# XinMing0411/zero-shot-AAC

Hardware: AMD Instinct MI355X
Metric: audio clips/sec end-to-end (encode+mapper+GPT-2 decode), Clotho-eval bs=64 (higher is better)
Workload: dtype bf16

## Files before the change

zero-shot-aac_amd/csrc/gemm.hip:

```cpp
#include <algorithm>
#include "gemm_fast.h"

namespace zs {

int g_gemm_fast = 1;
int g_gemm_dbg = 0;
int g_fast_xcd = 1;

__device__ __forceinline__ void store_out(void* out, int out_dtype, long idx, float v) {
  if (out_dtype == ZS_BF16) reinterpret_cast<bf16_t*>(out)[idx] = f2bf(v);
  else reinterpret_cast<float*>(out)[idx] = v;
}

template <typename T, int BM, int BN>
__global__ __launch_bounds__(256) void gemm_kernel(GemmArgs g) {
  constexpr int LDW = BK + GemmTraits<T>::PAD;
  __shared__ __attribute__((aligned(16))) T smem[2 * (BM + BN) * LDW];
  constexpr int TM = BM / 64, TN = BN / 64;
  const int n0 = blockIdx.x * BN, m0 = blockIdx.y * BM, z = blockIdx.z;
  const int kbeg = z * g.k_per_split, kend = min(g.K, kbeg + g.k_per_split);
  f32x16_t acc[TM][TN];
  DenseA<T, BM> la{(const T*)g.A, g.lda, g.M, m0};
  gemm_mainloop<T, BM, BN>(la, (const T*)g.W, g.ldw, g.N, n0, kbeg, kend, smem, acc);
  const int lane = threadIdx.x & 63, wid = threadIdx.x >> 6;
  const int wr0 = (wid >> 1) * (BM / 2), wc0 = (wid & 1) * (BN / 2);
#pragma unroll
  for (int i = 0; i < TM; ++i)
#pragma unroll
    for (int j = 0; j < TN; ++j) {
      const int n = n0 + wc0 + j * 32 + (lane & 31);
      if (n >= g.N) continue;
      const float bias = (g.split_k == 1 && g.bias) ? g.bias[n] : 0.f;
#pragma unroll
      for (int e = 0; e < 16; ++e) {
        const int m = m0 + wr0 + i * 32 + (e & 3) + 8 * (e >> 2) + 4 * (lane >> 5);
        if (m >= g.M) continue;
        float v = acc[i][j][e];
        if (g.split_k > 1) {
          g.ws[((long)z * g.M + m) * g.N + n] = v;
        } else {
          v = act_apply(v + bias, g.act);
          if (g.residual) v += g.residual[(long)m * g.ldr + n];
          store_out(g.out, g.out_dtype, (long)m * g.ldo + n, v);
        }
      }
    }
}

__global__ void splitk_reduce_kernel(GemmArgs g) {
  long idx = (long)blockIdx.x * blockDim.x + threadIdx.x;
  long total = (long)g.M * g.N;
  if (idx >= total) return;
  int m = idx / g.N, n = idx % g.N;
  float v = 0.f;
  for (int z = 0; z < g.split_k; ++z) v += g.ws[(long)z * total + idx];
  if (g.bias) v += g.bias[n];
  v = act_apply(v, g.act);
  if (g.residual) v += g.residual[(long)m * g.ldr + n];
  store_out(g.out, g.out_dtype, (long)m * g.ldo + n, v);
}

template <int ACT, int WN>
__device__ __forceinline__ void epi_slab(const GemmArgs& g, const float* slab, int mr0, int nc0,
                                         int z, bool vec_out, bool vec_res, const float (&bb)[8],
                                         const float4 (&res)[WN / 16][2]) {
  constexpr int Q = WN / 8, IT = 32 * Q / 64;
  static_assert(IT * 64 == 32 * Q, "slab iterations");
  const int lane = threadIdx.x & 63;
#pragma unroll
  for (int it = 0; it < IT; ++it) {
    const int idx = lane + 64 * it;
    const int r = idx / Q, c = (idx % Q) * 8;
    const int m = mr0 + r, n = nc0 + c;
    if (m >= g.M || n >= g.N) continue;
    const float4 a0 = *reinterpret_cast<const float4*>(slab + r * WN + c);
    const float4 a1 = *reinterpret_cast<const float4*>(slab + r * WN + c + 4);
    float v[8] = {a0.x, a0.y, a0.z, a0.w, a1.x, a1.y, a1.z, a1.w};
    const int nv = min(8, g.N - n);
    const bool full = nv == 8;
    if (g.split_k > 1) {
      float* dst = g.ws + ((long)z * g.M + m) * g.N + n;
      if (full && g.N % 4 == 0) {
        reinterpret_cast<float4*>(dst)[0] = make_float4(v[0], v[1], v[2], v[3]);
        reinterpret_cast<float4*>(dst)[1] = make_float4(v[4], v[5], v[6], v[7]);
      } else {
        for (int q = 0; q < nv; ++q) dst[q] = v[q];
      }
      continue;
    }
    if constexpr (64 % Q == 0) {
#pragma unroll
      for (int q = 0; q < 8; ++q) v[q] = act_apply_fast(v[q] + bb[q], ACT);
    } else {
#pragma unroll
      for (int q = 0; q < 8; ++q)
        v[q] = act_apply_fast(v[q] + ((g.bias && q < nv) ? g.bias[n + q] : 0.f), ACT);
    }
    if (g.residual) {
      if (full && vec_res) {
        const float4 r0 = res[it][0], r1 = res[it][1];
        v[0] += r0.x; v[1] += r0.y; v[2] += r0.z; v[3] += r0.w;
        v[4] += r1.x; v[5] += r1.y; v[6] += r1.z; v[7] += r1.w;
      } else {
        const float* rp = g.residual + (long)m * g.ldr + n;
        for (int q = 0; q < nv; ++q) v[q] += rp[q];
      }
    }
    const long o = (long)m * g.ldo + n;
    if (full && vec_out) {
      if (g.out_dtype == ZS_BF16) {
        uint4 u;
        u.x = pk2bf(v[0], v[1]);
        u.y = pk2bf(v[2], v[3]);
        u.z = pk2bf(v[4], v[5]);
        u.w = pk2bf(v[6], v[7]);
        if (g.dbg != 6 || u.x == 0x7fc17fc1u)
          *reinterpret_cast<uint4*>(reinterpret_cast<bf16_t*>(g.out) + o) = u;
      } else {
        float4* d = reinterpret_cast<float4*>(reinterpret_cast<float*>(g.out) + o);
        d[0] = make_float4(v[0], v[1], v[2], v[3]);
        d[1] = make_float4(v[4], v[5], v[6], v[7]);
      }
    } else {
      for (int q = 0; q < nv; ++q) store_out(g.out, g.out_dtype, o + q, v[q]);
    }
  }
}

template <int WN>
__device__ __forceinline__ void epi_res_load(const GemmArgs& g, int mr0, int nc0, bool vec_res,
                                             float4 (&res)[WN / 16][2]) {
  constexpr int Q = WN / 8, IT = 32 * Q / 64;
  const int lane = threadIdx.x & 63;
#pragma unroll
  for (int it = 0; it < IT; ++it) {
    const int idx = lane + 64 * it;
    const int m = mr0 + idx / Q, n = nc0 + (idx % Q) * 8;
    if (g.residual && vec_res && g.split_k == 1 && m < g.M && n + 8 <= g.N) {
      const float4* rp = reinterpret_cast<const float4*>(g.residual + (long)m * g.ldr + n);
      res[it][0] = rp[0];
      res[it][1] = rp[1];
    } else {
      res[it][0] = res[it][1] = make_float4(0.f, 0.f, 0.f, 0.f);
    }
  }
}

template <int BM, int BN, int NS, int WGM, int WGN, int BK_, bool F32 = false>
__global__ __launch_bounds__(64 * WGM * WGN,
                             (WGM * WGN == 4 && NS * FastTile<BM, BN, WGM, WGN, BK_>::STAGE <= 80 * 1024)
                                 ? 2 : 1) void gemm_fast_kernel(GemmArgs g) {
  constexpr int KF = F32 ? 2 : 1;
  using FT = FastTile<BM, BN, WGM, WGN, BK_>;
  __shared__ __attribute__((aligned(16))) char lds[NS * FT::STAGE];
  constexpr int TM = FT::TM, TN = FT::TN, WN = FT::WN;
  if (g.dbg == 5) return;
  static_assert(FT::NW * 32 * WN * 4 <= NS * FT::STAGE, "epilogue slab must fit the stage ring");
  const int ntn = cdiv(g.N, BN), ntm = cdiv(g.M, BM);
  const int ntiles = ntn * ntm * g.split_k;
// ... 87 lines not shown
      for (int q = 0; q < WN / 16; ++q) { res[q][0] = res0[q][0]; res[q][1] = res0[q][1]; }
    } else {
      epi_res_load<WN>(g, mr0, nc0, vec_res, res);
    }
#pragma unroll
    for (int j = 0; j < TN; ++j)
#pragma unroll
      for (int e = 0; e < 16; ++e)
        slab[((e & 3) + 8 * (e >> 2) + 4 * (lane >> 5)) * WN + j * 32 + (lane & 31)] = acc[i][j][e];
    switch (g.act) {
      case ACT_GELU_ERF: epi_slab<ACT_GELU_ERF, WN>(g, slab, mr0, nc0, cz, vec_out, vec_res, bb, res); break;
      case ACT_GELU_TANH: epi_slab<ACT_GELU_TANH, WN>(g, slab, mr0, nc0, cz, vec_out, vec_res, bb, res); break;
      case ACT_RELU: epi_slab<ACT_RELU, WN>(g, slab, mr0, nc0, cz, vec_out, vec_res, bb, res); break;
      case ACT_TANH: epi_slab<ACT_TANH, WN>(g, slab, mr0, nc0, cz, vec_out, vec_res, bb, res); break;
      default: epi_slab<ACT_NONE, WN>(g, slab, mr0, nc0, cz, vec_out, vec_res, bb, res); break;
    }
  }
  asm volatile("s_waitcnt lgkmcnt(0)" ::: "memory");
  __builtin_amdgcn_s_barrier();
  }
}

template <int BM, int BN, int NS, int BK_, int WGM = 2, int WGN = 2>
__global__ __launch_bounds__(64 * WGM * WGN, WGM * WGN == 4 ? 2 : 1) void gemm_lean_kernel(GemmArgs g) {
  using FT = FastTile<BM, BN, WGM, WGN, BK_>;
  constexpr int TM = FT::TM, TN = FT::TN, WN = FT::WN, NW = WGM * WGN;
  static_assert(NW * 32 * WN * 4 <= NS * FT::STAGE, "epilogue slab fits the ring");
  __shared__ __attribute__((aligned(16))) char lds[NS * FT::STAGE];
  const int ntn = cdiv(g.N, BN), ntm = cdiv(g.M, BM), ntiles = ntn * ntm;
  int m0, n0;
  {
    const int b = blockIdx.x, x = b & 7, q8 = ntiles >> 3, r8 = ntiles & 7;
    const int u = (x < r8 ? x * (q8 + 1) : r8 * (q8 + 1) + (x - r8) * q8) + (b >> 3);
    const int conc = max(1, min(q8, 64));
    int gm = (int)(sqrtf((float)conc * BN / BM) + 0.5f);
    gm = max(1, min(gm, ntm));
    const int per = gm * ntn, grp = u / per, fm = grp * gm;
    const int gs = min(ntm - fm, gm), r = u - grp * per;
    m0 = (fm + r % gs) * BM;
    n0 = (r / gs) * BN;
  }
  const int lane = threadIdx.x & 63, wid = threadIdx.x >> 6;
  f32x16_t acc[TM][TN];
  lean_mainloop<BM, BN, NS, WGM, WGN, BK_, false, true>((const bf16_t*)g.A, g.lda, g.M, m0,
                                                        (const bf16_t*)g.W, g.ldw, g.N, n0, g.K,
                                                        lds, acc);
  const int wr0 = (wid / WGN) * FT::WM, wc0 = (wid % WGN) * WN;
  const bool vec_out = g.ldo % 8 == 0 && ((uintptr_t)g.out & 15) == 0;
  const bool vec_res = g.residual == nullptr || (g.ldr % 4 == 0 && ((uintptr_t)g.residual & 15) == 0);
  float bb[8];
  {
    const int n = n0 + wc0 + (lane % (WN / 8)) * 8, nv = min(8, g.N - n);
    if (g.bias && nv == 8 && ((uintptr_t)(g.bias + n) & 15) == 0) {
      const float4 b0 = reinterpret_cast<const float4*>(g.bias + n)[0];
      const float4 b1 = reinterpret_cast<const float4*>(g.bias + n)[1];
      bb[0] = b0.x; bb[1] = b0.y; bb[2] = b0.z; bb[3] = b0.w;
      bb[4] = b1.x; bb[5] = b1.y; bb[6] = b1.z; bb[7] = b1.w;
    } else {
#pragma unroll
      for (int q = 0; q < 8; ++q) bb[q] = (g.bias && q < nv) ? g.bias[n + q] : 0.f;
    }
  }
  float* slab = reinterpret_cast<float*>(lds) + wid * 32 * WN;
#pragma unroll
  for (int i = 0; i < TM; ++i) {
    const int mr0 = m0 + wr0 + i * 32, nc0 = n0 + wc0;
    float4 res[WN / 16][2];
    epi_res_load<WN>(g, mr0, nc0, vec_res, res);
#pragma unroll
    for (int j = 0; j < TN; ++j)
#pragma unroll
      for (int e = 0; e < 16; ++e)
        slab[((e & 3) + 8 * (e >> 2) + 4 * (lane >> 5)) * WN + j * 32 + (lane & 31)] = acc[i][j][e];
    switch (g.act) {
      case ACT_GELU_ERF: epi_slab<ACT_GELU_ERF, WN>(g, slab, mr0, nc0, 0, vec_out, vec_res, bb, res); break;
      case ACT_GELU_TANH: epi_slab<ACT_GELU_TANH, WN>(g, slab, mr0, nc0, 0, vec_out, vec_res, bb, res); break;
      case ACT_RELU: epi_slab<ACT_RELU, WN>(g, slab, mr0, nc0, 0, vec_out, vec_res, bb, res); break;
      case ACT_TANH: epi_slab<ACT_TANH, WN>(g, slab, mr0, nc0, 0, vec_out, vec_res, bb, res); break;
      default: epi_slab<ACT_NONE, WN>(g, slab, mr0, nc0, 0, vec_out, vec_res, bb, res); break;
    }
  }
}

namespace big {
constexpr int BM = 256, BN = 256, BKB = 64, RB = 128, BUF = (BM + BN) * RB;
__device__ __forceinline__ int swz(int row) { return (row >> 1) & 7; }
__device__ __forceinline__ int set_instr(int set, int j) {
  if (set < 2) return ((j >> 3) * 128 + set * 64) / 8 + (j & 7);
  return (BM + (j >> 2) * 64 + (set - 2) * 32) / 8 + (j & 3);
}
}

typedef __attribute__((ext_vector_type(4))) float f32x4_t;
template <int ACT>
__device__ __forceinline__ void big_epilogue(const GemmArgs& g, float* slab, int mrw, int nc0,
                                             bool vec_out, bool vec_res, const float (&bb)[8],
                                             const f32x4_t (&acc)[8][4]) {
  const int lane = threadIdx.x & 63, fr = lane & 15, fq = lane >> 4;
#pragma unroll
  for (int sl = 0; sl < 4; ++sl) {
    const int mr0 = mrw + 32 * sl;
    float4 res[4][2];
    epi_res_load<64>(g, mr0, nc0, vec_res, res);
#pragma unroll
    for (int ii = 0; ii < 2; ++ii)
#pragma unroll
      for (int j = 0; j < 4; ++j)
#pragma unroll
        for (int e = 0; e < 4; ++e)
          slab[(16 * ii + 4 * fq + e) * 64 + 16 * j + fr] = acc[2 * sl + ii][j][e];
    epi_slab<ACT, 64>(g, slab, mr0, nc0, 0, vec_out, vec_res, bb, res);
  }
}

__global__ __launch_bounds__(512) void gemm_big_kernel(GemmArgs g) {
  using namespace big;
  __shared__ __attribute__((aligned(16))) char lds[2 * BUF];
  const int ntn = cdiv(g.N, BN), ntm = cdiv(g.M, BM), ntiles = ntn * ntm;
  int m0, n0;
  {
    const int b = blockIdx.x, x = b & 7, q8 = ntiles >> 3, r8 = ntiles & 7;
    const int u = (x < r8 ? x * (q8 + 1) : r8 * (q8 + 1) + (x - r8) * q8) + (b >> 3);
    const int conc = max(1, min(q8, 32));
    int gm = (int)(sqrtf((float)conc) + 0.5f);
    gm = max(1, min(gm, ntm));
    const int per = gm * ntn, grp = u / per, fm = grp * gm;
    const int gs = min(ntm - fm, gm), r = u - grp * per;
    m0 = (fm + r % gs) * BM;
    n0 = (r / gs) * BN;
  }
  const int lane = threadIdx.x & 63, wid = threadIdx.x >> 6, wr = wid >> 2, wc = wid & 3;
  const bf16_t* A = (const bf16_t*)g.A;
  const bf16_t* W = (const bf16_t*)g.W;
  int src[4][2];
#pragma unroll
  for (int set = 0; set < 4; ++set)
#pragma unroll
    for (int jj = 0; jj < 2; ++jj) {
      const int idx = set_instr(set, wid + 8 * jj);
      const int row = 8 * idx + (lane >> 3);
      const int c = 8 * ((lane & 7) ^ swz(row));
      src[set][jj] = set < 2 ? min(m0 + row, g.M - 1) * g.lda + c
                             : min(n0 + row - BM, g.N - 1) * g.ldw + c;
    }
  auto issue = [&](int set, char* bufp, int k0) {
#pragma unroll
    for (int jj = 0; jj < 2; ++jj)
      __builtin_amdgcn_global_load_lds((gptr_t)((set < 2 ? A : W) + src[set][jj] + k0),
                                       (lds_ptr_t)(bufp + set_instr(set, wid + 8 * jj) * 1024),
                                       16, 0, 0);
  };
  auto tile_issue = [&](char* bufp, int k0) {
    issue(0, bufp, k0); issue(2, bufp, k0); issue(3, bufp, k0); issue(1, bufp, k0);
  };
  f32x4_t acc[8][4];
#pragma unroll
  for (int i = 0; i < 8; ++i)
#pragma unroll
    for (int j = 0; j < 4; ++j) acc[i][j] = f32x4_t{0.f, 0.f, 0.f, 0.f};
  const int nk = g.K / BKB;
  tile_issue(lds, 0);
  if (nk > 1) tile_issue(lds + BUF, BKB);
  const int fr = lane & 15, fq = lane >> 4;
  const int arow = wr * 128 + fr, brow = BM + wc * 64 + fr;
  int aoff[2], boff[2];
#pragma unroll
  for (int s2 = 0; s2 < 2; ++s2) {
    aoff[s2] = arow * RB + 16 * ((4 * s2 + fq) ^ swz(arow));
    boff[s2] = brow * RB + 16 * ((4 * s2 + fq) ^ swz(brow));
  }
  bf16x8_t a[4][2], b0[2][2], b1[2][2];
#pragma unroll 1
  for (int t = 0; t < nk; ++t) {
    char* bufp = lds + (t & 1) * BUF;
    const bool pf = t + 2 < nk;
    const int kn = (t + 2) * BKB;
// ... 38 lines not shown
          acc[i][2 + j] = __builtin_amdgcn_mfma_f32_16x16x32_bf16(a[i][s2], b1[j][s2], acc[i][2 + j], 0, 0, 0);
    __builtin_amdgcn_s_setprio(0);
    if (pf) wait_vm<12>(); else if (t + 2 == nk) wait_vm<8>(); else wait_vm<0>();
    __builtin_amdgcn_s_barrier();
    asm volatile("" ::: "memory");
#pragma unroll
    for (int i = 0; i < 4; ++i)
#pragma unroll
      for (int s2 = 0; s2 < 2; ++s2)
        a[i][s2] = *reinterpret_cast<const bf16x8_t*>(bufp + aoff[s2] + 2048 * (4 + i));
    if (pf) issue(3, bufp, kn);
    __builtin_amdgcn_s_setprio(1);
#pragma unroll
    for (int s2 = 0; s2 < 2; ++s2)
#pragma unroll
      for (int i = 0; i < 4; ++i)
#pragma unroll
        for (int j = 0; j < 2; ++j)
          acc[4 + i][2 + j] = __builtin_amdgcn_mfma_f32_16x16x32_bf16(a[i][s2], b1[j][s2], acc[4 + i][2 + j], 0, 0, 0);
    __builtin_amdgcn_s_setprio(0);
    __builtin_amdgcn_s_barrier();
    asm volatile("" ::: "memory");
    if (pf) issue(1, bufp, kn);
    __builtin_amdgcn_s_setprio(1);
#pragma unroll
    for (int s2 = 0; s2 < 2; ++s2)
#pragma unroll
      for (int i = 0; i < 4; ++i)
#pragma unroll
        for (int j = 0; j < 2; ++j)
          acc[4 + i][j] = __builtin_amdgcn_mfma_f32_16x16x32_bf16(a[i][s2], b0[j][s2], acc[4 + i][j], 0, 0, 0);
    __builtin_amdgcn_s_setprio(0);
  }
  wait_vm<0>();
  __syncthreads();
  const bool vec_out = g.ldo % 8 == 0 && ((uintptr_t)g.out & 15) == 0;
  const bool vec_res = g.residual == nullptr || (g.ldr % 4 == 0 && ((uintptr_t)g.residual & 15) == 0);
  const int nc0 = n0 + wc * 64;
  float bb[8];
  {
    const int n = nc0 + (lane % 8) * 8, nv = min(8, g.N - n);
    if (g.bias && nv == 8 && ((uintptr_t)(g.bias + n) & 15) == 0) {
      const float4 c0 = reinterpret_cast<const float4*>(g.bias + n)[0];
      const float4 c1 = reinterpret_cast<const float4*>(g.bias + n)[1];
      bb[0] = c0.x; bb[1] = c0.y; bb[2] = c0.z; bb[3] = c0.w;
      bb[4] = c1.x; bb[5] = c1.y; bb[6] = c1.z; bb[7] = c1.w;
    } else {
#pragma unroll
      for (int q = 0; q < 8; ++q) bb[q] = (g.bias && q < nv) ? g.bias[n + q] : 0.f;
    }
  }
  float* slab = reinterpret_cast<float*>(lds) + wid * 32 * 64;
  const int mrw = m0 + wr * 128;
  switch (g.act) {
    case ACT_GELU_ERF: big_epilogue<ACT_GELU_ERF>(g, slab, mrw, nc0, vec_out, vec_res, bb, acc); break;
    case ACT_GELU_TANH: big_epilogue<ACT_GELU_TANH>(g, slab, mrw, nc0, vec_out, vec_res, bb, acc); break;
    case ACT_RELU: big_epilogue<ACT_RELU>(g, slab, mrw, nc0, vec_out, vec_res, bb, acc); break;
    case ACT_TANH: big_epilogue<ACT_TANH>(g, slab, mrw, nc0, vec_out, vec_res, bb, acc); break;
    default: big_epilogue<ACT_NONE>(g, slab, mrw, nc0, vec_out, vec_res, bb, acc); break;
  }
}

int g_gemm_big = 1;
int g_big_min = 256;

static int launch_big(GemmArgs& g, hipStream_t st) {
  hipLaunchKernelGGL(gemm_big_kernel, dim3(cdiv(g.N, 256) * cdiv(g.M, 256)), dim3(512), 0, st, g);
  ZS_LAUNCH_CHECK();
  return 0;
}

int g_gemm_lean = 1;
int g_lean96 = 0;
int g_lean8w = 0;

template <int BM, int BN, int NS, int BK_, int WGM = 2, int WGN = 2>
static int launch_lean(GemmArgs& g, hipStream_t st) {
  hipLaunchKernelGGL((gemm_lean_kernel<BM, BN, NS, BK_, WGM, WGN>),
                     dim3(cdiv(g.N, BN) * cdiv(g.M, BM)), dim3(64 * WGM * WGN), 0, st, g);
  ZS_LAUNCH_CHECK();
  return 0;
}

int g_fast_persist = 1;

template <int BM, int BN, int NS, int WGM = 2, int WGN = 2, int BK_ = 64, bool F32 = false>
static int launch_fast(GemmArgs& g, hipStream_t st) {
  using FT = FastTile<BM, BN, WGM, WGN, BK_>;
  const long nt = (long)cdiv(g.N, BN) * cdiv(g.M, BM) * g.split_k;
  const int per_cu = max(1, min(160 * 1024 / (NS * FT::STAGE), 8 / FT::NW * 2));
  dim3 grid(g_fast_persist ? (int)std::min<long>(nt, 256L * per_cu) : (int)nt);
  hipLaunchKernelGGL((gemm_fast_kernel<BM, BN, NS, WGM, WGN, BK_, F32>), grid,
                     dim3(64 * WGM * WGN), 0, st, g);
  ZS_LAUNCH_CHECK();
  return 0;
}

static long nblocks(const GemmArgs& g, int bm, int bn) {
  return (long)cdiv(g.M, bm) * cdiv(g.N, bn) * g.split_k;
}

int g_fast_ns = 2;
int g_fast_tile = 0;
int g_lean_min128 = 256;
#ifndef ZS_LEAN128_NS
#define ZS_LEAN128_NS 3
#endif
int g_lean128_ns = ZS_LEAN128_NS;

static int dispatch_fast(GemmArgs& g, hipStream_t st) {
  switch (g_fast_tile) {
    case 1: return launch_fast<256, 256, 4, 2, 4, 32>(g, st);
    case 2: return launch_fast<256, 128, 4, 4, 2, 32>(g, st);
    case 3: return launch_fast<128, 256, 4, 2, 4, 32>(g, st);
    case 4: return launch_fast<128, 128, 2>(g, st);
    case 5: return launch_fast<128, 128, 4, 2, 2, 32>(g, st);
    case 6: return launch_fast<256, 256, 2, 2, 4, 64>(g, st);
    case 7: return launch_fast<128, 128, 6, 2, 2, 32>(g, st);
    case 8: return launch_fast<128, 64, 3>(g, st);
    case 9: return launch_fast<64, 128, 3>(g, st);
    case 10: return launch_fast<128, 128, 3>(g, st);
    case 11: return launch_fast<128, 128, 2, 2, 2, 32>(g, st);
    case 12: return launch_fast<128, 128, 3, 2, 2, 32>(g, st);
    case 13: return launch_fast<64, 64, 2>(g, st);
    case 14: return launch_fast<128, 128, 4>(g, st);
    case 15: return launch_fast<256, 128, 2, 4, 2, 64>(g, st);
    case 16: return launch_fast<128, 256, 2, 2, 4, 64>(g, st);
    case 17: return launch_fast<64, 64, 2, 2, 2, 128>(g, st);
    default: break;
  }
  if ((g_fast_tile == 18 || (g_gemm_big && g.K >= 2048 && nblocks(g, 256, 256) >= g_big_min)) &&
      g.split_k == 1 && g.K % 64 == 0 && g.lda % 8 == 0 && g.ldw % 8 == 0)
    return launch_big(g, st);
  if (g_gemm_lean && g.split_k == 1 && g.K % 64 == 0) {
    const int lt = g_fast_tile >= 100 ? g_fast_tile - 100 : 0;
    const long n128 = nblocks(g, 128, 128);
    if (!lt && g_lean8w && g.N >= 3072 && n128 >= 1024 && n128 <= 4096)
      return launch_lean<256, 128, 3, 64, 2, 4>(g, st);
    if (!lt && g_lean96 && g.N % 96 == 0 && g.N <= 1536 && nblocks(g, 128, 96) >= 384)
      return launch_lean<128, 96, 2, 64, 4, 1>(g, st);
    if (lt == 1 || (!lt && n128 >= g_lean_min128)) return launch_lean<128, 128, 2, 64>(g, st);
    if (!lt && n128 >= 128)
      return g_lean128_ns == 4 ? launch_lean<128, 128, 4, 64, 2, 4>(g, st)
                               : launch_lean<128, 128, 3, 64, 2, 4>(g, st);
    if (lt == 2 || (!lt && nblocks(g, 128, 64) >= 256))
      return g.M >= g.N ? launch_lean<128, 64, 3, 64>(g, st) : launch_lean<64, 128, 3, 64>(g, st);
    if ((lt == 3 || (!lt && g.M >= 512 && nblocks(g, 64, 64) < 256)) && g.K % 128 == 0)
      return launch_lean<64, 64, 2, 128>(g, st);
    if (lt == 5) return launch_lean<256, 128, 2, 64, 4, 2>(g, st);
    if (lt == 6) return launch_lean<128, 256, 2, 64, 2, 4>(g, st);
    if (lt == 7) return launch_lean<256, 256, 2, 64, 2, 4>(g, st);
    if (lt == 8) return launch_lean<256, 128, 3, 64, 4, 2>(g, st);
    if (lt == 9) return launch_lean<128, 256, 3, 64, 2, 4>(g, st);
    if (lt == 10) return launch_lean<256, 128, 3, 64, 2, 4>(g, st);
    if (lt == 11) return launch_lean<128, 128, 3, 64, 2, 4>(g, st);
    if (lt == 12) return launch_lean<128, 128, 4, 64, 2, 4>(g, st);
    if (lt == 13) return launch_lean<128, 96, 2, 64, 4, 1>(g, st);
    return launch_lean<64, 64, 4, 64>(g, st);
  }
  if (nblocks(g, 128, 128) >= 256) {
    if (g_fast_ns == 3) return launch_fast<128, 128, 3>(g, st);
    if (g_fast_ns == 4) return launch_fast<128, 128, 4>(g, st);
    return launch_fast<128, 128, 2>(g, st);
  }
  if (nblocks(g, 128, 64) >= 256) return g.M >= g.N ? launch_fast<128, 64, 3>(g, st)
                                                     : launch_fast<64, 128, 3>(g, st);
  if (g.k_per_split % 128 == 0) return launch_fast<64, 64, 2, 2, 2, 128>(g, st);
  return launch_fast<64, 64, 4>(g, st);
}

template <typename T, int BM, int BN>
static int launch_gemm(GemmArgs& g, hipStream_t st) {
  dim3 grid(cdiv(g.N, BN), cdiv(g.M, BM), g.split_k);
  hipLaunchKernelGGL((gemm_kernel<T, BM, BN>), grid, dim3(256), 0, st, g);
  ZS_LAUNCH_CHECK();
  return 0;
}

int g_f32_fast = 1;
int g_f32_tile = 8;
static int dispatch_fast_f32(GemmArgs& g, hipStream_t st) {
  if (g_f32_tile >= 7) {
    if (nblocks(g, 128, 128) >= 256) {
      if (g_f32_tile == 10) return launch_fast<128, 128, 2, 2, 2, 128, true>(g, st);
      if (g_f32_tile == 11 && nblocks(g, 256, 128) >= 256)
        return launch_fast<256, 128, 2, 4, 2, 64, true>(g, st);
      return g_f32_tile == 7 ? launch_fast<128, 128, 2, 2, 4, 64, true>(g, st)
                             : launch_fast<128, 128, 2, 2, 2, 64, true>(g, st);
    }
    if (nblocks(g, 128, 64) >= 256)
      return g.M >= g.N ? launch_fast<128, 64, 2, 2, 2, 64, true>(g, st)
                        : launch_fast<64, 128, 2, 2, 2, 64, true>(g, st);
    return launch_fast<64, 64, 2, 2, 2, 64, true>(g, st);
  }
  if (g_f32_tile && nblocks(g, 128, 128) >= 256) {
    switch (g_f32_tile) {
      case 1: return launch_fast<128, 128, 3, 2, 2, 64, true>(g, st);
      case 2: return launch_fast<128, 128, 2, 2, 2, 64, true>(g, st);
      case 3: return launch_fast<256, 128, 4, 4, 2, 32, true>(g, st);
      case 4: return launch_fast<128, 256, 4, 2, 4, 32, true>(g, st);
      case 5: return launch_fast<128, 128, 6, 2, 2, 32, true>(g, st);
      case 6: return launch_fast<128, 128, 4, 2, 4, 32, true>(g, st);
      default: break;
    }
  }
  if (nblocks(g, 128, 128) >= 256) return launch_fast<128, 128, 4, 2, 2, 32, true>(g, st);
  if (nblocks(g, 128, 64) >= 256)
    return g.M >= g.N ? launch_fast<128, 64, 4, 2, 2, 32, true>(g, st)
                      : launch_fast<64, 128, 4, 2, 2, 32, true>(g, st);
  return launch_fast<64, 64, 4, 2, 2, 32, true>(g, st);
}

template <typename T>
static int dispatch_gemm(GemmArgs& g, hipStream_t st) {
  if (sizeof(T) == 2 && g_gemm_fast) return dispatch_fast(g, st);
  if (sizeof(T) == 4 && g_f32_fast && g.K % 4 == 0 && g.lda % 4 == 0 && g.ldw % 4 == 0 &&
      g.k_per_split % 4 == 0 && ((uintptr_t)g.A & 15) == 0 && ((uintptr_t)g.W & 15) == 0)
    return dispatch_fast_f32(g, st);
  const bool small_m = g.M <= 64;
  const bool wide_n = g.N >= 2048 && !small_m;
  if (small_m) return wide_n ? launch_gemm<T, 64, 128>(g, st) : launch_gemm<T, 64, 64>(g, st);
  if (wide_n) return launch_gemm<T, 128, 128>(g, st);
  return launch_gemm<T, 128, 64>(g, st);
}

}

using namespace zs;

extern "C" __attribute__((visibility("hidden"))) int zs_gemm_skinny_internal(
    int M, int N, int K, int dtype, const void* A, int lda, const void* W, int ldw,
    const float* bias, const float* residual, int ldr, void* out, int ldo, int out_dtype, int act,
    float* workspace, void* stream);

extern "C" __attribute__((visibility("hidden"))) int zs_gemm_rows_internal(
    int M, int N, int K, const void* A, int lda, const void* W, int ldw, const float* bias,
    const float* residual, int ldr, void* out, int ldo, int out_dtype, int act, void* stream);

extern "C" int zs_gemm(int M, int N, int K, int dtype, const void* A, int lda, const void* W,
                       int ldw, const float* bias, const float* residual, int ldr, void* out,
// ... 44 lines not shown
```

zero-shot-aac_amd/csrc/gemm_skinny.hip:

```cpp
#include <cstring>
#include "common.h"

namespace zs {

typedef __attribute__((ext_vector_type(8))) __bf16 bf16x8s_t;
typedef __attribute__((ext_vector_type(16))) float f32x16s_t;

constexpr int SK_BN = 32;
constexpr int SK_TILE = 64 * SK_BN;
constexpr int SK_MAX_TILES = 4096;
constexpr int SK_MAX_M = 256;

struct SkinnyArgs {
  int M, N, K, lda, ldw, ldr, ldo, splits, ks;
  int rblocks, ntiles;
  const void* A;
  const void* W;
  const float* bias;
  const float* residual;
  void* out;
  int out_dtype, act;
  int* counters;
  float* slabs;
};
// ... 118 lines not shown
  }
  const int ntiles = g.ntiles;
  float* slabs = g.slabs + (long)rb * g.splits * ntiles * SK_TILE;
  int* counter = g.counters + rb * ntiles + tile;
  const long slab_off = ((long)z * ntiles + tile) * SK_TILE + e0;
  __amdgpu_buffer_rsrc_t rsrc = __builtin_amdgcn_make_buffer_rsrc(
      slabs, (short)0, g.splits * ntiles * SK_TILE * 4, 0x00020000);
  if (MODE == 1) {
#pragma unroll
    for (int q = 0; q < PER / 4; ++q) {
      u32x4_t v = {__float_as_uint(part[4 * q]), __float_as_uint(part[4 * q + 1]),
                   __float_as_uint(part[4 * q + 2]), __float_as_uint(part[4 * q + 3])};
      __builtin_amdgcn_raw_buffer_store_b128(v, rsrc, (int)((slab_off + 4 * q) * 4), 0, 16);
    }
  } else {
#pragma unroll
    for (int q = 0; q < PER / 4; ++q)
      *reinterpret_cast<float4*>(slabs + slab_off + 4 * q) =
          make_float4(part[4 * q], part[4 * q + 1], part[4 * q + 2], part[4 * q + 3]);
  }
  asm volatile("s_waitcnt vmcnt(0)" ::: "memory");
  __syncthreads();
  int* flag = reinterpret_cast<int*>(red + 4 * SK_TILE);
  if (threadIdx.x == 0) {
    if (MODE == 0) {
      __builtin_amdgcn_fence(__ATOMIC_RELEASE, "agent");
      asm volatile("s_waitcnt vmcnt(0)" ::: "memory");
    }
    const int old = __hip_atomic_fetch_add(counter, 1, __ATOMIC_RELAXED, __HIP_MEMORY_SCOPE_AGENT);
    const int last = old == g.splits - 1;
    if (last) {
      __hip_atomic_store(counter, 0, __ATOMIC_RELAXED, __HIP_MEMORY_SCOPE_AGENT);
      if (MODE == 0) {
        __builtin_amdgcn_fence(__ATOMIC_ACQUIRE, "agent");
        asm volatile("s_waitcnt vmcnt(0)" ::: "memory");
      }
    }
    *flag = last;
  }
  __syncthreads();
  if (!*flag) return;
  float v[PER];
#pragma unroll
  for (int i = 0; i < PER; ++i) v[i] = 0.f;
  for (int s = 0; s < g.splits; ++s) {
    const long off = ((long)s * ntiles + tile) * SK_TILE + e0;
#pragma unroll
    for (int q = 0; q < PER / 4; ++q) {
      float4 f;
      if (MODE == 1) {
        const u32x4_t u = __builtin_amdgcn_raw_buffer_load_b128(rsrc, (int)((off + 4 * q) * 4), 0, 16);
        f = make_float4(__uint_as_float(u.x), __uint_as_float(u.y), __uint_as_float(u.z),
                        __uint_as_float(u.w));
      } else {
        f = *reinterpret_cast<const float4*>(slabs + off + 4 * q);
      }
      v[4 * q] += f.x; v[4 * q + 1] += f.y; v[4 * q + 2] += f.z; v[4 * q + 3] += f.w;
    }
  }
#pragma unroll
  for (int i = 0; i < PER; ++i)
    if (m < Mr && nb + i < g.N) skinny_store(g, rb * 64 + m, nb + i, v[i]);
}

static int g_skinny_mode = 1;
extern int g_gemm_fast;
extern int g_f32_fast;
extern int g_decode_attn5;
extern int g_window_mfma;
extern int g_fast_ns;
extern int g_fast_tile;
extern int g_gemm_dbg;
extern int g_fast_persist;
extern int g_fast_xcd;
extern int g_swin_dbg;
extern int g_swin_occ3;
extern int g_gemm_lean;
extern int g_row_mfma;
extern int g_logmel_wave;
extern int g_lean96;
extern int g_lean8w;
extern int g_lean_min128;
extern int g_lean128_ns;
extern int g_lm_prio;
extern int g_gemm_rows;
extern int g_rows_nt48;
extern int g_fp8_tile;
extern int g_rows_wide;
extern int g_fp8_dbg;
extern int g_attn_split;
extern int g_small_attn;
extern int g_small_rmax;
extern int g_gemm_big;
extern int g_big_min;
extern int g_dp_spin;
extern int g_dp_abort;
extern int g_dg_exp;
extern int g_dg_dynf;
extern int g_beam_xcd;
extern int g_f32_tile;

static int skinny_splits(int N, int K) {
  const int ntiles = cdiv(N, SK_BN);
  int best = -1;
  for (int s = 1; s <= K / 64; ++s) {
    if (K % s) continue;
    const int ks = K / s;
    if (ks % 64 || ks > 512) continue;
    if (best < 0) best = s;
    if (ntiles * s >= 256) { best = s; break; }
    best = s;
  }
  return best;
}

}

using namespace zs;

extern "C" int zs_tune_set(const char* key, int value) {
  if (!key) return ZS_ERR_ARG;
  if (!strcmp(key, "skinny_mode")) { g_skinny_mode = value; return 0; }
  if (!strcmp(key, "gemm_fast")) { g_gemm_fast = value; return 0; }
  if (!strcmp(key, "f32_fast")) { g_f32_fast = value; return 0; }
  if (!strcmp(key, "decode_attn5")) {
    if (value == 0 || value == 1 || value == 5)
      return fail(ZS_ERR_ARG, "zs_tune_set: decode_attn5 = %d chose a kernel that is retired "
                  "(6, 4, 3 or 2: decode_attn6's phase length and reductions)", value);
    ZS_REQUIRE(value == 2 || value == 3 || value == 4 || value == 6,
               "zs_tune_set: decode_attn5 = %d (6, 4, 3 or 2)", value);
    g_decode_attn5 = value;
    return 0;
  }
  if (!strcmp(key, "window_mfma")) { g_window_mfma = value; return 0; }
  if (!strcmp(key, "fast_ns")) { g_fast_ns = value; return 0; }
  if (!strcmp(key, "fast_tile")) { g_fast_tile = value; return 0; }
  if (!strcmp(key, "gemm_dbg")) { g_gemm_dbg = value; return 0; }
  if (!strcmp(key, "fast_persist")) { g_fast_persist = value; return 0; }
  if (!strcmp(key, "fast_xcd")) { g_fast_xcd = value; return 0; }
  if (!strcmp(key, "swin_dbg")) { g_swin_dbg = value; return 0; }
  if (!strcmp(key, "swin_occ3")) { g_swin_occ3 = value; return 0; }
  if (!strcmp(key, "gemm_lean")) { g_gemm_lean = value; return 0; }
  if (!strcmp(key, "row_mfma")) { g_row_mfma = value; return 0; }
  if (!strcmp(key, "logmel_wave")) { g_logmel_wave = value; return 0; }
  if (!strcmp(key, "lean96")) { g_lean96 = value; return 0; }
  if (!strcmp(key, "lean8w")) { g_lean8w = value; return 0; }
  if (!strcmp(key, "lean_min128")) { g_lean_min128 = value; return 0; }
  if (!strcmp(key, "lean128_ns")) { g_lean128_ns = value; return 0; }
  if (!strcmp(key, "lm_prio")) { g_lm_prio = value; return 0; }
  if (!strcmp(key, "gemm_rows")) { g_gemm_rows = value; return 0; }
  if (!strcmp(key, "rows_nt48")) { g_rows_nt48 = value; return 0; }
  if (!strcmp(key, "fp8_tile")) { g_fp8_tile = value; return 0; }
  if (!strcmp(key, "rows_wide")) { g_rows_wide = value; return 0; }
  if (!strcmp(key, "fp8_dbg")) { g_fp8_dbg = value; return 0; }
  if (!strcmp(key, "attn_split")) { g_attn_split = value; return 0; }
  if (!strcmp(key, "small_attn")) { g_small_attn = value; return 0; }
  if (!strcmp(key, "small_rmax")) { g_small_rmax = value; return 0; }
  if (!strcmp(key, "gemm_big")) { g_gemm_big = value; return 0; }
  if (!strcmp(key, "big_min")) { g_big_min = value; return 0; }
  if (!strcmp(key, "dp_spin")) { g_dp_spin = value; return 0; }
  if (!strcmp(key, "dp_abort_step")) { g_dp_abort = value; return 0; }
  if (!strcmp(key, "dg_exp")) { g_dg_exp = value; return 0; }
  if (!strcmp(key, "dg_dynf")) { g_dg_dynf = value; return 0; }
  if (!strcmp(key, "beam_xcd")) { g_beam_xcd = value; return 0; }
  if (!strcmp(key, "f32_tile")) { g_f32_tile = value; return 0; }
  return fail(ZS_ERR_ARG, "zs_tune_set: unknown key %s", key);
}

extern "C" int zs_gemm_workspace_floats(int M, int N, int K) {
  if (M <= 0 || M > SK_MAX_M) return 0;
  const int s = skinny_splits(N, K);
  if (s < 0) return 0;
  const int ntiles = cdiv(N, SK_BN), rb = cdiv(M, 64);
  if (ntiles * rb > SK_MAX_TILES) return 0;
  return SK_MAX_TILES + rb * s * ntiles * SK_TILE;
}

extern "C" __attribute__((visibility("hidden"))) int zs_gemm_skinny_internal(int M, int N, int K, int dtype, const void* A, int lda,
                                       const void* W, int ldw, const float* bias,
                                       const float* residual, int ldr, void* out, int ldo,
                                       int out_dtype, int act, float* workspace, void* stream) {
  ZS_REQUIRE(M > 0 && M <= SK_MAX_M, "skinny gemm: M <= %d", SK_MAX_M);
  const int s = skinny_splits(N, K);
  ZS_REQUIRE(s > 0, "skinny gemm: K=%d must be a multiple of 64", K);
  const int ntiles = cdiv(N, SK_BN), rb = cdiv(M, 64);
  ZS_REQUIRE(s == 1 || workspace != nullptr, "skinny gemm: needs the zeroed workspace");
  ZS_REQUIRE(ntiles * rb <= SK_MAX_TILES, "skinny gemm: N too large");
  SkinnyArgs g{M, N, K, lda, ldw, ldr, ldo, s, K / s, rb, ntiles, A, W, bias, residual, out,
               out_dtype, act, reinterpret_cast<int*>(workspace), workspace + SK_MAX_TILES};
  dim3 grid(ntiles * s * rb);
#define SKL(T, MODE_) hipLaunchKernelGGL((gemm_skinny_kernel<T, MODE_>), grid, dim3(256), 0, S(stream), g)
  if (dtype == ZS_BF16) {
    if (g_skinny_mode == 1) SKL(bf16_t, 1); else SKL(bf16_t, 0);
  } else {
    if (g_skinny_mode == 1) SKL(float, 1); else SKL(float, 0);
  }
#undef SKL
  ZS_LAUNCH_CHECK();
  return 0;
}
```

Measured before the change: 8001.

## Add persistent ring-buffered lean GEMM overlapping next-tile prefetch with epilogue

Adds a persistent 128x128 GEMM kernel that walks tiles with an XCD-aware grouped schedule. It prefetches the next tile's first K stages, plus its bias and residual, while the current tile's epilogue runs, reusing LDS stages outside the epilogue slab. The kernel runs two workgroups per CU and uses counted vmcnt waits and raw ds_read in the epilogue. Ring mode 5 (2 stages, BK=64) becomes the default for the large lean path, which adds code complexity and raises LDS-aliasing and synchronisation risk.

```diff
diff --git a/zero-shot-aac_amd/csrc/gemm.hip b/zero-shot-aac_amd/csrc/gemm.hip
--- a/zero-shot-aac_amd/csrc/gemm.hip
+++ b/zero-shot-aac_amd/csrc/gemm.hip
@@ -60,7 +60,7 @@
   store_out(g.out, g.out_dtype, (long)m * g.ldo + n, v);
 }
 
-template <int ACT, int WN>
+template <int ACT, int WN, bool RAWRD = false>
 __device__ __forceinline__ void epi_slab(const GemmArgs& g, const float* slab, int mr0, int nc0,
                                          int z, bool vec_out, bool vec_res, const float (&bb)[8],
                                          const float4 (&res)[WN / 16][2]) {
@@ -73,8 +73,15 @@
     const int r = idx / Q, c = (idx % Q) * 8;
     const int m = mr0 + r, n = nc0 + c;
     if (m >= g.M || n >= g.N) continue;
-    const float4 a0 = *reinterpret_cast<const float4*>(slab + r * WN + c);
-    const float4 a1 = *reinterpret_cast<const float4*>(slab + r * WN + c + 4);
+    float4 a0, a1;
+    if constexpr (RAWRD) {
+      const unsigned ad = (unsigned)(uintptr_t)(lds_ptr_t)(void*)(slab + r * WN + c);
+      asm volatile("ds_read_b128 %0, %2\n\tds_read_b128 %1, %2 offset:16\n\ts_waitcnt lgkmcnt(0)"
+                   : "=&v"(a0), "=&v"(a1) : "v"(ad) : "memory");
+    } else {
+      a0 = *reinterpret_cast<const float4*>(slab + r * WN + c);
+      a1 = *reinterpret_cast<const float4*>(slab + r * WN + c + 4);
+    }
     float v[8] = {a0.x, a0.y, a0.z, a0.w, a1.x, a1.y, a1.z, a1.w};
     const int nv = min(8, g.N - n);
     const bool full = nv == 8;
@@ -328,6 +335,190 @@
   }
 }
 
+typedef __attribute__((ext_vector_type(4))) float f32x4_t;
+template <int NS, int BK_>
+__global__ __launch_bounds__(256, 2) void gemm_lean_ring_kernel(GemmArgs g) {
+  constexpr int BM = 128, BN = 128;
+  using FT = FastTile<BM, BN, 2, 2, BK_>;
+  constexpr int TM = FT::TM, TN = FT::TN, WN = FT::WN, NW = FT::NW, IPW = FT::NI / NW;
+  constexpr int SL = NW * 32 * WN * 4 / FT::STAGE;
+  constexpr int P = NS - SL;
+  constexpr int XS = TM * (32 * (WN / 8) / 64);
+  static_assert(NS >= 2 && (NS - 2) * IPW + XS < 64, "counted waits");
+  static_assert(SL * FT::STAGE == NW * 32 * WN * 4 && P >= 1 && P <= NS - 1,
+                "the epilogue slab is whole stages and leaves one to prefetch into");
+  static_assert(NS * FT::STAGE <= 80 * 1024, "two workgroups per CU");
+  static_assert(BM / FT::RPI % NW == 0, "a wave's j-th DMA instruction is A rows or W rows for all waves");
+  __shared__ __attribute__((aligned(16))) char lds[NS * FT::STAGE];
+  const int ntn = cdiv(g.N, BN), ntm = cdiv(g.M, BM), ntiles = ntn * ntm;
+  const int lane = threadIdx.x & 63, wid = threadIdx.x >> 6;
+  const int q8 = ntiles >> 3, r8 = ntiles & 7;
+  int gm = (int)(sqrtf((float)max(1, min(q8, 64)) * BN / BM) + 0.5f);
+  gm = max(1, min(gm, ntm));
+  auto tile = [&](int t, int& m0, int& n0) {
+    const int x = t & 7;
+    const int u = (x < r8 ? x * (q8 + 1) : r8 * (q8 + 1) + (x - r8) * q8) + (t >> 3);
+    const int per = gm * ntn, grp = u / per, fm = grp * gm;
+    const int gs = min(ntm - fm, gm), r = u - grp * per;
+    m0 = (fm + r % gs) * BM;
+    n0 = (r / gs) * BN;
+  };
+  unsigned src[IPW];
+  auto point = [&](int m0, int n0) {
+    const int rsub = lane / FT::SPR, slot = lane % FT::SPR;
+#pragma unroll
+    for (int j = 0; j < IPW; ++j) {
+      const int row = FT::RPI * (wid + NW * j) + rsub;
+      const int c = 8 * (slot ^ FT::swz(row));
+      if (NW * j < BM / FT::RPI) src[j] = 2u * ((unsigned)min(m0 + row, g.M - 1) * g.lda + c);
+      else src[j] = 2u * ((unsigned)min(n0 + row - BM, g.N - 1) * g.ldw + c);
+    }
+  };
+  auto issue = [&](int stage, int k0) {
+#pragma unroll
+    for (int j = 0; j < IPW; ++j) {
+      const char* base = reinterpret_cast<const char*>(NW * j < BM / FT::RPI ? g.A : g.W) + 2 * k0;
+      __builtin_amdgcn_global_load_lds((gptr_t)(base + src[j]),
+                                       (lds_ptr_t)(lds + stage * FT::STAGE + (wid + NW * j) * 1024),
+                                       16, 0, 0);
+    }
+  };
+  const int nk = g.K / BK_;
+  const int wr0 = (wid / 2) * FT::WM, wc0 = (wid % 2) * WN;
+  const bool vec_out = g.ldo % 8 == 0 && ((uintptr_t)g.out & 15) == 0;
+  const bool vec_res = g.residual == nullptr || (g.ldr % 4 == 0 && ((uintptr_t)g.residual & 15) == 0);
+  float* slab = reinterpret_cast<float*>(lds + P * FT::STAGE) + wid * 32 * WN;
+  constexpr int Q = WN / 8, IT = 32 * Q / 64;
+  f32x4_t braw[2];
+  float4 res[TM][IT][2];
+#pragma unroll
+  for (int h = 0; h < 2; ++h) {
+    braw[h] = f32x4_t{0.f, 0.f, 0.f, 0.f};
+#pragma unroll
+    for (int i = 0; i < TM; ++i)
+#pragma unroll
+      for (int it = 0; it < IT; ++it) res[i][it][h] = make_float4(0.f, 0.f, 0.f, 0.f);
+  }
+  auto full_tile = [&](int m0, int n0) { return m0 + BM <= g.M && n0 + BN <= g.N; };
+  auto bias_pre = [&](int m0, int n0) {
+    return g.bias && ((uintptr_t)g.bias & 15) == 0 && full_tile(m0, n0);
+  };
+  auto res_pre = [&](int m0, int n0) { return g.residual && vec_res && full_tile(m0, n0); };
+  auto load_epi = [&](int m0, int n0) {
+    if (bias_pre(m0, n0)) {
+      const f32x4_t* bp = reinterpret_cast<const f32x4_t*>(g.bias + n0 + wc0 + (lane % Q) * 8);
+      braw[0] = bp[0];
+      braw[1] = bp[1];
+    }
+    if (res_pre(m0, n0)) {
+      const float* rt = g.residual + (long)m0 * g.ldr + n0;
+#pragma unroll
+      for (int i = 0; i < TM; ++i)
+#pragma unroll
+        for (int it = 0; it < IT; ++it) {
+          const int idx = lane + 64 * it;
+          const float4* rp = reinterpret_cast<const float4*>(
+              rt + (wr0 + i * 32 + idx / Q) * g.ldr + wc0 + (idx % Q) * 8);
+          res[i][it][0] = rp[0];
+          res[i][it][1] = rp[1];
+        }
+    }
+  };
+  auto landed = [&]() {
+#pragma unroll
+    for (int h = 0; h < 2; ++h) asm volatile("" ::"v"(braw[h]));
+#pragma unroll
+    for (int i = 0; i < TM; ++i)
+#pragma unroll
+      for (int it = 0; it < IT; ++it)
+#pragma unroll
+        for (int h = 0; h < 2; ++h)
+          asm volatile("" ::"v"(res[i][it][h].x), "v"(res[i][it][h].y), "v"(res[i][it][h].z),
+                       "v"(res[i][it][h].w));
+  };
+  int t = blockIdx.x, m0, n0;
+  tile(t, m0, n0);
+  point(m0, n0);
+  load_epi(m0, n0);
+#pragma unroll
+  for (int p = 0; p < NS - 1; ++p)
+    if (p < nk) issue(p, p * BK_);
+  bool xs = false;
+  for (;;) {
+    f32x16_t acc[TM][TN];
+#pragma unroll
+    for (int i = 0; i < TM; ++i)
+#pragma unroll
+      for (int j = 0; j < TN; ++j)
+#pragma unroll
+        for (int e = 0; e < 16; ++e) acc[i][j][e] = 0.f;
+    int st = 0, kt = 0;
+    if (xs) {
+      for (; kt < min(P, nk); ++kt) {
+        if (kt + NS - 2 < nk) wait_vm<(NS - 2) * IPW + XS>(); else wait_vm<XS>();
+        __builtin_amdgcn_s_barrier();
+        if (kt + NS - 1 < nk) issue(st == 0 ? NS - 1 : st - 1, (kt + NS - 1) * BK_);
+        fast_compute<BM, BN, 2, 2, BK_, false, true>(lds + st * FT::STAGE, acc);
+        st = st == NS - 1 ? 0 : st + 1;
+      }
+    }
+    for (; kt < nk; ++kt) {
+      if (kt + NS - 2 < nk) wait_vm<(NS - 2) * IPW>(); else wait_vm<0>();
+      __builtin_amdgcn_s_barrier();
+      if (kt + NS - 1 < nk) issue(st == 0 ? NS - 1 : st - 1, (kt + NS - 1) * BK_);
+      fast_compute<BM, BN, 2, 2, BK_, false, true>(lds + st * FT::STAGE, acc);
+      st = st == NS - 1 ? 0 : st + 1;
+    }
+    asm volatile("s_waitcnt lgkmcnt(0)" ::: "memory");
+    __builtin_amdgcn_s_barrier();
+    landed();
+    const int cm0 = m0, cn0 = n0;
+    const bool cres = res_pre(cm0, cn0);
+    float bb[8] = {braw[0].x, braw[0].y, braw[0].z, braw[0].w, braw[1].x, braw[1].y, braw[1].z, braw[1].w};
+    if (!bias_pre(cm0, cn0)) {
+      const int n = cn0 + wc0 + (lane % Q) * 8, nv = min(8, g.N - n);
+#pragma unroll
+      for (int q = 0; q < 8; ++q) bb[q] = (g.bias && q < nv) ? g.bias[n + q] : 0.f;
+    }
+#pragma unroll
+    for (int q = 0; q < 8; ++q) asm volatile("" ::"v"(bb[q]));
+    const int tn = t + (int)gridDim.x;
+    const bool more = tn < ntiles;
+    if (more) {
+      tile(tn, m0, n0);
+      point(m0, n0);
+#pragma unroll
+      for (int p = 0; p < P; ++p)
+        if (p < nk) issue(p, p * BK_);
+    }
+#pragma unroll
+    for (int i = 0; i < TM; ++i) {
+      const int mr0 = cm0 + wr0 + i * 32, nc0 = cn0 + wc0;
+#pragma unroll
+      for (int j = 0; j < TN; ++j)
+#pragma unroll
+        for (int e = 0; e < 16; ++e)
+          slab[((e & 3) + 8 * (e >> 2) + 4 * (lane >> 5)) * WN + j * 32 + (lane & 31)] = acc[i][j][e];
+      switch (g.act) {
+        case ACT_GELU_ERF: epi_slab<ACT_GELU_ERF, WN, true>(g, slab, mr0, nc0, 0, vec_out, cres, bb, res[i]); break;
+        case ACT_GELU_TANH: epi_slab<ACT_GELU_TANH, WN, true>(g, slab, mr0, nc0, 0, vec_out, cres, bb, res[i]); break;
+        case ACT_RELU: epi_slab<ACT_RELU, WN, true>(g, slab, mr0, nc0, 0, vec_out, cres, bb, res[i]); break;
+        case ACT_TANH: epi_slab<ACT_TANH, WN, true>(g, slab, mr0, nc0, 0, vec_out, cres, bb, res[i]); break;
+        default: epi_slab<ACT_NONE, WN, true>(g, slab, mr0, nc0, 0, vec_out, cres, bb, res[i]); break;
+      }
+    }
+    if (!more) break;
+    asm volatile("s_waitcnt lgkmcnt(0)" ::: "memory");
+    __builtin_amdgcn_s_barrier();
+    load_epi(m0, n0);
+#pragma unroll
+    for (int p = P; p < NS - 1; ++p)
+      if (p < nk) issue(p, p * BK_);
+    xs = g.dbg != 6 && cm0 + BM <= g.M && cn0 + BN <= g.N;
+    t = tn;
+  }
+}
+
 namespace big {
 constexpr int BM = 256, BN = 256, BKB = 64, RB = 128, BUF = (BM + BN) * RB;
 __device__ __forceinline__ int swz(int row) { return (row >> 1) & 7; }
@@ -337,7 +528,6 @@
 }
 }
 
-typedef __attribute__((ext_vector_type(4))) float f32x4_t;
 template <int ACT>
 __device__ __forceinline__ void big_epilogue(const GemmArgs& g, float* slab, int mrw, int nc0,
                                              bool vec_out, bool vec_res, const float (&bb)[8],
@@ -542,6 +732,17 @@
   return 0;
 }
 
+template <int NS, int BK_>
+static int launch_lean_ring(GemmArgs& g, hipStream_t st) {
+  const long nt = (long)cdiv(g.N, 128) * cdiv(g.M, 128);
+  if ((long)g.M * g.lda >= (1L << 31) || (long)g.N * g.ldw >= (1L << 31))
+    return launch_lean<128, 128, 2, 64>(g, st);
+  hipLaunchKernelGGL((gemm_lean_ring_kernel<NS, BK_>), dim3((int)std::min<long>(nt, 2 * 256)), dim3(256),
+                     0, st, g);
+  ZS_LAUNCH_CHECK();
+  return 0;
+}
+
 int g_fast_persist = 1;
 
 template <int BM, int BN, int NS, int WGM = 2, int WGN = 2, int BK_ = 64, bool F32 = false>
@@ -563,6 +764,7 @@
 int g_fast_ns = 2;
 int g_fast_tile = 0;
 int g_lean_min128 = 256;
+int g_lean_ring = 5;
 #ifndef ZS_LEAN128_NS
 #define ZS_LEAN128_NS 3
 #endif
@@ -599,7 +801,16 @@
       return launch_lean<256, 128, 3, 64, 2, 4>(g, st);
     if (!lt && g_lean96 && g.N % 96 == 0 && g.N <= 1536 && nblocks(g, 128, 96) >= 384)
       return launch_lean<128, 96, 2, 64, 4, 1>(g, st);
-    if (lt == 1 || (!lt && n128 >= g_lean_min128)) return launch_lean<128, 128, 2, 64>(g, st);
+    if (lt == 1 || (!lt && n128 >= g_lean_min128)) {
+      switch (lt ? 0 : g_lean_ring) {
+        case 1: return launch_lean<128, 128, 4, 32>(g, st);
+        case 2: return launch_lean<128, 128, 5, 32>(g, st);
+        case 3: return launch_lean_ring<4, 32>(g, st);
+        case 4: return launch_lean_ring<5, 32>(g, st);
+        case 5: return launch_lean_ring<2, 64>(g, st);
+        default: return launch_lean<128, 128, 2, 64>(g, st);
+      }
+    }
     if (!lt && n128 >= 128)
       return g_lean128_ns == 4 ? launch_lean<128, 128, 4, 64, 2, 4>(g, st)
                                : launch_lean<128, 128, 3, 64, 2, 4>(g, st);
@@ -616,6 +827,11 @@
     if (lt == 11) return launch_lean<128, 128, 3, 64, 2, 4>(g, st);
     if (lt == 12) return launch_lean<128, 128, 4, 64, 2, 4>(g, st);
     if (lt == 13) return launch_lean<128, 96, 2, 64, 4, 1>(g, st);
+    if (lt == 14) return launch_lean<128, 128, 4, 32>(g, st);
+    if (lt == 15) return launch_lean<128, 128, 5, 32>(g, st);
+    if (lt == 16) return launch_lean_ring<4, 32>(g, st);
+    if (lt == 17) return launch_lean_ring<5, 32>(g, st);
+    if (lt == 18) return launch_lean_ring<2, 64>(g, st);
     return launch_lean<64, 64, 4, 64>(g, st);
   }
   if (nblocks(g, 128, 128) >= 256) {
diff --git a/zero-shot-aac_amd/csrc/gemm_skinny.hip b/zero-shot-aac_amd/csrc/gemm_skinny.hip
--- a/zero-shot-aac_amd/csrc/gemm_skinny.hip
+++ b/zero-shot-aac_amd/csrc/gemm_skinny.hip
@@ -224,6 +224,7 @@
 extern int g_lean8w;
 extern int g_lean_min128;
 extern int g_lean128_ns;
+extern int g_lean_ring;
 extern int g_lm_prio;
 extern int g_gemm_rows;
 extern int g_rows_nt48;
@@ -289,6 +290,7 @@
   if (!strcmp(key, "lean8w")) { g_lean8w = value; return 0; }
   if (!strcmp(key, "lean_min128")) { g_lean_min128 = value; return 0; }
   if (!strcmp(key, "lean128_ns")) { g_lean128_ns = value; return 0; }
+  if (!strcmp(key, "lean_ring")) { g_lean_ring = value; return 0; }
   if (!strcmp(key, "lm_prio")) { g_lm_prio = value; return 0; }
   if (!strcmp(key, "gemm_rows")) { g_gemm_rows = value; return 0; }
   if (!strcmp(key, "rows_nt48")) { g_rows_nt48 = value; return 0; }
```

After: 7946. No clear change (-0.7%).
